# ontypehq/libfst

Hardware: AMD Instinct MI355X
Metric: strings/sec, compose_frozen_shortest_path_ambiguous len=64 batch=1M (higher is better)
Workload: dtype f64; 1 GPU; compose_frozen_shortest_path_ambiguous; semantics=eager, len=64, transducer_len=4096, branches=12, strings_per_gpu=1048576, global_batch=1048576, scaling_mode=weak: 1048576 strings per GPU per step, parallelism=dp1 (string shards, rhs replicated via RCCL broadcast)

## Files before the change

### libfst_amd/csrc/device_engine.hpp

```cpp
#pragma once

#include <hip/hip_runtime.h>

#include <atomic>
#include <condition_variable>
#include <cstdint>
#include <mutex>
#include <new>
#include <vector>

#include "fst_core.hpp"

namespace fstamd {

class FrozenFst;

constexpr uint32_t kSpanMixed = 0xFFFFFFFEu;
constexpr uint32_t kSpanNone = 0xFFFFFFFFu;
constexpr uint32_t kRecPad = 16;
constexpr uint32_t kDeadLabel = 0xFFFFFFFFu;

struct RhsView {
  const uint2* span;
  const double* final_w;
  const uint32_t* il;
  const ArcRec* rec;
  const uint4* sspan;
  uint32_t num_states;
  uint32_t num_arcs;
  uint32_t start;
  uint32_t max_span;
  uint32_t jump_back;
  uint32_t jump_fwd;
  const uint4* sspan2;
};

constexpr uint32_t kRevPos = 0x1000u;
struct RevRec {
  uint32_t src;
  uint32_t y;
  double weight;
};
static_assert(sizeof(RevRec) == 16, "RevRec is one 16-byte load");
struct RevView {
  const uint4* rspan;
  const uint4* gtab;
  const RevRec* rrec;
  const uint32_t* rolab;
  uint32_t kp;
  uint32_t gsearch;
  uint32_t direct;
  const uint4* rrec32;
  const uint2* rrec8;
  const uint32_t* rlab;
  const uint2* rxrec;
  uint32_t nrec;
  const uint32_t* rrec4;
  uint32_t rbias8;
  double winv;
};
constexpr uint32_t kPullWt = 64;
constexpr uint32_t kPullWtMax = 256;
__host__ __device__ inline const double* rv_weight_table(const RevView& rv) {
  return reinterpret_cast<const double*>(rv.rrec4 + ((rv.nrec + 1u) & ~1u));
}
constexpr double kRec8WMax = 7.0;

struct DeviceFst {
  int dev = 0;
  uint8_t* blob = nullptr;
  size_t blob_size = 0;
  uint2* span = nullptr;
  double* final_w = nullptr;
  uint32_t* il = nullptr;
  ArcRec* rec = nullptr;
  uint4* sspan = nullptr;
  RhsView view{};
  bool has_eps = false;
  bool nonneg = true;
  bool nan = false;
  bool finite = true;
  uint8_t weight_type = 0;
  bool pull_ok = false;
  bool lazy_pull_ok = false;
  double int_wmax = -1.0;
  bool widx = false;
  uint32_t wt_n = 0;
  bool byte_back = false;
  mutable std::atomic<int> skip_tiny_lazy{0}, skip_tiny_eager{0};
  mutable std::atomic<int> tiny_lazy_256{0}, tiny_eager_256{0};
  mutable std::atomic<uint64_t> tiny_lazy_seen{0}, tiny_lazy_over{0};
  RevView rev{};
  void* rev_bufs[9] = {};
  uint32_t* band_il = nullptr;
  ArcRec* band_rec = nullptr;
  uint32_t band_sh = 0;
  bool band_ol_sorted = false;
  std::vector<uint32_t> perm;

  static DeviceFst* create(const FrozenFst& f, int dev);
  static DeviceFst* adopt(const void* d_blob, const FrozenFst& host_view, int dev);
  static void destroy(DeviceFst* d);
};

struct BatchOutDev {
  int32_t* status;
  uint32_t* path_len;
  uint64_t* path_off;
  double* final_w;
  uint32_t* out_il;
  uint32_t* out_ol;
  double* out_w;
  uint64_t arc_cap;
  unsigned long long* cursor;
  uint32_t* work;
  const uint64_t* slots = nullptr;
  uint32_t* host_ol = nullptr;
  double* host_w = nullptr;
  int32_t* first_status = nullptr;
};

struct ChainInput {
  const uint32_t* labels;
  const uint64_t* offsets;
  uint32_t num_strings;
  uint32_t max_len;
};
struct GraphInput {
  const uint32_t* state_off;
  const uint32_t* arc_il;
  const uint32_t* arc_ol;
  const double* arc_w;
  const uint32_t* arc_next;
  const double* final_w;
  uint32_t num_states;
  uint32_t start;
  uint32_t max_outdeg;
  uint32_t ncap;
  uint32_t eps_out;
};

void* pin_host_alloc(size_t bytes);
void pin_host_release(void* p);
void device_pool_release(int dev);
template <class T>
struct PinnedAllocator {
  using value_type = T;
  PinnedAllocator() = default;
  template <class U>
  PinnedAllocator(const PinnedAllocator<U>&) {}
  T* allocate(size_t n) {
    void* p = pin_host_alloc(n * sizeof(T));
    if (!p) throw std::bad_alloc();
    return (T*)p;
  }
  void deallocate(T* p, size_t) { pin_host_release(p); }
  template <class U>
  bool operator==(const PinnedAllocator<U>&) const { return true; }
  template <class U>
  bool operator!=(const PinnedAllocator<U>&) const { return false; }
};
template <class T>
using PinnedVec = std::vector<T, PinnedAllocator<T>>;

struct HostLattice {
  int32_t status = 0;
  uint32_t n_nodes = 0, n_arcs = 0;
  PinnedVec<uint32_t> aoff, anext, ail, aol;
  PinnedVec<double> aw, nfin;
};
// ... 140 lines not shown
```

### libfst_amd/csrc/eager_pull.hip

```cpp
#include <algorithm>
#include <cmath>
#include <cstdio>
#include <cstdlib>
#include <cstring>
#include <unordered_map>
#include <vector>

#include "device_engine.hpp"
#include "host_fst.hpp"
#include "kernels/eager_pull.hpp"
#include "kernels/lazy_pull.hpp"

namespace fstamd {

namespace {

template <int KP, int WV, int RK>
const void* pull_kernel_ptr(bool direct) {
  return direct ? (const void*)eager_pull_kernel<kPullRows, KP, true, WV, RK>
                : (const void*)eager_pull_kernel<kPullRows, KP, false, WV, RK>;
}
#ifndef FSTAMD_PULL_WAVES_SMALL
#define FSTAMD_PULL_WAVES_SMALL 5
#endif
#ifndef FSTAMD_PULL_WAVES_F32
#define FSTAMD_PULL_WAVES_F32 6
#endif
#ifndef FSTAMD_PULL_WAVES_R8
#define FSTAMD_PULL_WAVES_R8 7
#endif
template <int RK>
const void* pull_kernel_for(const RevView& rv) {
  const bool dir = rv.direct != 0;
  constexpr int wv = RK == 5 ? 4
                   : RK == 4 ? FSTAMD_PULL_WAVES_SMALL
                   : RK >= 2 ? FSTAMD_PULL_WAVES_R8 : RK ? FSTAMD_PULL_WAVES_F32 : FSTAMD_PULL_WAVES_SMALL;
  switch (rv.kp) {
    case 4: return pull_kernel_ptr<4, wv, RK>(dir);
    case 5: return pull_kernel_ptr<5, wv, RK>(dir);
    default: return pull_kernel_ptr<8, 4, RK>(dir);
  }
}
bool use_rec8(const RevView& rv) { return rv.rrec8 && !std::getenv("FSTAMD_NO_REC8"); }
int route_rk(const char* sem, int rk, const RevView& rv, bool log) {
  if (log && std::getenv("FSTAMD_ROUTE_LOG"))
    std::fprintf(stderr, "[libfst_amd route] %s pull: records %d, weight scale %g\n", sem, rk,
                 rk && rk < 4 ? 1.0 / rv.winv : 1.0);
  return rk;
}
int pull_rk(const DeviceFst& rhs, uint32_t max_len) {
  if (!pull_f32(rhs, max_len) || std::getenv("FSTAMD_P_F64"))
    return rhs.rev.rrec4 && rhs.widx && !std::getenv("FSTAMD_NO_REC4")
               ? (rhs.wt_n <= kPullWt ? 4 : 5)
               : 0;
  if (rhs.rev.rrec4 && use_rec8(rhs.rev) && !std::getenv("FSTAMD_NO_REC4")) return 3;
  return use_rec8(rhs.rev) ? 2 : 1;
}
const void* pull_kernel_for(const DeviceFst& rhs, uint32_t max_len, bool log = false) {
  switch (route_rk("eager", pull_rk(rhs, max_len), rhs.rev, log)) {
    case 0: return pull_kernel_for<0>(rhs.rev);
    case 5: return pull_kernel_for<5>(rhs.rev);
    case 4: return pull_kernel_for<4>(rhs.rev);
    case 3: return pull_kernel_for<3>(rhs.rev);
    case 2: return pull_kernel_for<2>(rhs.rev);
    default: return pull_kernel_for<1>(rhs.rev);
  }
}
#ifndef FSTAMD_LP_WAVES_F32
#define FSTAMD_LP_WAVES_F32 5
#endif
#ifndef FSTAMD_LP_WAVES_F64
#define FSTAMD_LP_WAVES_F64 4
#endif
constexpr int kLazyPullWaves = 3;
template <int KP, int RK>
const void* lazy_pull_ptr(bool direct, bool b1) {
  constexpr int wv = KP > 5 ? kLazyPullWaves
                   : RK ? FSTAMD_LP_WAVES_F32 : FSTAMD_LP_WAVES_F64;
  if (!direct) return (const void*)lazy_pull_kernel<kPullRows, KP, false, wv, RK, false>;
  return b1 ? (const void*)lazy_pull_kernel<kPullRows, KP, true, wv, RK, true>
            : (const void*)lazy_pull_kernel<kPullRows, KP, true, wv, RK, false>;
}
template <int RK>
const void* lazy_pull_kernel_for(const DeviceFst& rhs) {
  const bool dir = rhs.rev.direct != 0, b1 = dir && rhs.byte_back;
  switch (rhs.rev.kp) {
    case 4: return lazy_pull_ptr<4, RK>(dir, b1);
    case 5: return lazy_pull_ptr<5, RK>(dir, b1);
    default: return lazy_pull_ptr<8, RK>(dir, b1);
  }
}
const void* lazy_pull_kernel_for(const DeviceFst& rhs, uint32_t max_len, bool log = false) {
  const int rk = !lazy_pull_f32(rhs, max_len) ? 0 : use_rec8(rhs.rev) ? 2 : 1;
  if (log && std::getenv("FSTAMD_ROUTE_LOG"))
    std::fprintf(stderr, "[libfst_amd route] lazy pull: back records %d B\n",
                 rhs.rev.direct && rhs.byte_back ? 1 : 4);
  switch (route_rk("lazy", rk, rhs.rev, log)) {
    case 0: return lazy_pull_kernel_for<0>(rhs);
    case 2: return lazy_pull_kernel_for<2>(rhs);
    default: return lazy_pull_kernel_for<1>(rhs);
  }
}
}

void free_reverse_mirror(DeviceFst* d) {
  for (void*& p : d->rev_bufs) {
    if (p) (void)hipFree(p);
    p = nullptr;
  }
  d->rev = RevView{};
  d->pull_ok = false;
  d->widx = false;
  d->wt_n = 0;
}

bool build_reverse_mirror(DeviceFst* d, const FrozenFst& f) {
  d->pull_ok = false;
  d->lazy_pull_ok = false;
  if (std::getenv("FSTAMD_NO_PULL")) return true;
  if (d->has_eps || !d->nonneg || d->nan) return true;
  const uint32_t ns = f.num_states(), na = f.header().num_arcs;
  if (ns == 0 || ns >= (1u << 27)) return true;
  const StateEntry* se = f.states();
  const PackedArc* pa = f.arcs();
  const std::vector<uint32_t>& perm = d->perm;
  auto pid = [&](uint32_t s) { return perm.empty() ? s : perm[s]; };

  std::vector<uint8_t> jpos(na);
  std::vector<uint32_t> src(na);
  std::vector<uint32_t> indeg(ns + 1, 0);
  for (uint32_t s = 0; s < ns; ++s) {
    uint32_t run = se[s].arc_offset;
    for (uint32_t a = se[s].arc_offset; a < se[s].arc_offset + se[s].num_arcs; ++a) {
      if (a > se[s].arc_offset && pa[a].ilabel != pa[a - 1].ilabel) run = a;
      if (a - run >= 8) return true;
      jpos[a] = (uint8_t)(a - run);
      src[a] = pid(s);
      ++indeg[pid(pa[a].nextstate)];
    }
  }
  bool ol_ordered = true;
  for (uint32_t s = 0; s < ns && ol_ordered; ++s)
    for (uint32_t a = se[s].arc_offset; a < se[s].arc_offset + se[s].num_arcs && ol_ordered; ++a)
      for (uint32_t b = a - jpos[a]; b < a; ++b)
        if (pa[b].nextstate == pa[a].nextstate && pa[b].olabel > pa[a].olabel) {
          ol_ordered = false;
          break;
        }
  std::vector<uint32_t> ioff(ns + 1, 0);
  for (uint32_t t = 0; t < ns; ++t) ioff[t + 1] = ioff[t] + indeg[t];
  std::vector<uint32_t> in(na), fill(ioff.begin(), ioff.end() - 1);
  for (uint32_t a = 0; a < na; ++a) in[fill[pid(pa[a].nextstate)]++] = a;
  for (uint32_t t = 0; t < ns; ++t)
    std::sort(in.begin() + ioff[t], in.begin() + ioff[t + 1], [&](uint32_t x, uint32_t y) {
      if (pa[x].ilabel != pa[y].ilabel) return pa[x].ilabel < pa[y].ilabel;
      if (src[x] != src[y]) return src[x] < src[y];
      return jpos[x] < jpos[y];
    });
  struct Group { uint32_t t, label, first, n; };
  std::vector<Group> groups;
  for (uint32_t t = 0; t < ns; ++t)
    for (uint32_t i = ioff[t]; i < ioff[t + 1];) {
      uint32_t e = i + 1;
      while (e < ioff[t + 1] && pa[in[e]].ilabel == pa[in[i]].ilabel) ++e;
      groups.push_back(Group{t, pa[in[i]].ilabel, i, e - i});
      i = e;
    }
  uint32_t kp = 8;
  uint64_t best_cost = ~0ull;
  for (uint32_t cand : {4u, 5u, 8u}) {
    uint64_t cost = 0;
    for (const Group& g : groups) {
      const uint64_t nb = (g.n + cand - 1) / cand;
      cost += nb * cand + (nb - 1) * cand;
    }
    if (cost < best_cost) {
      best_cost = cost;
      kp = cand;
    }
  }
  bool direct = !std::getenv("FSTAMD_PULL_INDIRECT");
  for (size_t g = 0; g < groups.size() && direct; ++g)
    if ((g > 0 && groups[g].t == groups[g - 1].t) || groups[g].label >= (1u << 24)) direct = false;
  const uint64_t ndirect = direct ? (uint64_t)ns + kPullW : 0;
  uint64_t nblocks = direct ? ndirect : 1;
  for (const Group& g : groups) nblocks += (g.n + kp - 1) / kp - (direct ? 1 : 0);
  if (nblocks * kp * sizeof(RevRec) > (4ull << 30) || nblocks * kp >= 0xFFFFFFFFull) return true;

  std::vector<RevRec> rrec(nblocks * kp, RevRec{0xFFFFFFF8u, 0u, 0.0});
  std::vector<uint32_t> rtgt(nblocks * kp, 0u);
  std::vector<uint32_t> rolab(nblocks * kp, 0u);
  std::vector<uint4> rspan((size_t)ns + kPullW, make_uint4(0u, 0u, kSpanNone, 0u));
  std::vector<uint4> gtab;
  uint32_t max_groups = 0;
  uint64_t blk = direct ? ndirect : 1;
  for (size_t gi = 0; gi < groups.size();) {
// ... 45 lines not shown
  for (uint32_t a = 0; a < na && d->int_wmax >= 0.0; ++a)
    d->int_wmax = std::max(d->int_wmax, pa[a].weight * wscale);
  if (wscale == 0.0) wscale = 1.0;
  auto wsc = [wscale](double w) { return (uint32_t)(w * wscale); };
  std::vector<uint32_t> rlab;
  std::vector<uint2> rxrec;
  if (direct) {
    rlab.resize(rspan.size());
    rxrec.resize(rspan.size());
    for (size_t t = 0; t < rspan.size(); ++t) {
      rlab[t] = (rspan[t].z & 0xFFFFFFu) | (std::min<uint32_t>(rspan[t].y, 255u) << 24);
      rxrec[t] = make_uint2(rspan[t].x, rspan[t].y);
    }
  }
  uint64_t max_nb = 0;
  for (const uint4& r : rspan)
    if (r.z != kSpanMixed) max_nb = std::max<uint64_t>(max_nb, r.y);
  const bool byte_back = direct && max_nb * kp <= 255 && !std::getenv("FSTAMD_NO_BYTE_BACK");
  std::vector<uint4> rrec32;
  std::vector<uint2> rrec8;
  if (d->int_wmax >= 0.0 && d->int_wmax <= kRec8WMax) {
    rrec8.resize(rrec.size());
    for (size_t r = 0; r < rrec.size(); ++r)
      rrec8[r] = make_uint2(rrec[r].src, rrec[r].y | wsc(rrec[r].weight));
  }
  std::vector<double> wtab;
  std::unordered_map<uint64_t, uint32_t> widx_of;
  if (d->int_wmax < 0.0 && !std::getenv("FSTAMD_NO_WIDX")) {
    bool ok = true;
    for (uint32_t a = 0; a < na && ok; ++a) {
      const double w = pa[a].weight;
      uint64_t bits;
      std::memcpy(&bits, &w, 8);
      if (widx_of.count(bits)) continue;
      if (!(w >= 0.0) || !std::isfinite(w) || wtab.size() == kPullWtMax) ok = false;
      else {
        widx_of.emplace(bits, (uint32_t)wtab.size());
        wtab.push_back(w);
      }
    }
    if (!ok) {
      wtab.clear();
      widx_of.clear();
    }
  }
  const bool widx = !wtab.empty();
  auto low_weight = [&](double w) -> uint32_t {
    if (!widx) return wsc(w);
    uint64_t bits;
    std::memcpy(&bits, &w, 8);
    return widx_of.at(bits);
  };
  std::vector<uint32_t> rrec4;
  uint32_t rbias8 = 0;
  if (!rrec8.empty() || widx) {
    int64_t dlo = 0, dhi = 0;
    for (size_t r = 0; r < rrec.size(); ++r) {
      if (rrec[r].src == 0xFFFFFFF8u) continue;
      const int64_t dl = (int64_t)rtgt[r] - (int64_t)(rrec[r].src >> 3);
      dlo = std::min(dlo, dl);
      dhi = std::max(dhi, dl);
    }
    if ((dhi - dlo) * 8 < 0xFFF0 && -dlo * 8 + 8 * (int64_t)kPullW <= 0xFFFF && byte_back) {
      rbias8 = (uint32_t)(-dlo * 8);
      rrec4.resize(rrec.size());
      for (size_t r = 0; r < rrec.size(); ++r) {
        const uint32_t y = rrec[r].y;
        if (rrec[r].src == 0xFFFFFFF8u) {
          rrec4[r] = 0xFFFF0000u;
        } else {
          const uint32_t low = (((y >> 17) & 7u) << 13) | (((y >> 13) & 15u) << 9) |
                               (((y >> 12) & 1u) << 8) | low_weight(rrec[r].weight);
          const int64_t dl = (int64_t)rtgt[r] - (int64_t)(rrec[r].src >> 3);
          rrec4[r] = ((uint32_t)((dl - dlo) * 8) << 16) | low;
        }
      }
    }
  }
  if (d->int_wmax >= 0.0) {
    rrec32.resize(rrec.size());
    for (size_t r = 0; r < rrec.size(); ++r)
      rrec32[r] = make_uint4(rrec[r].src, rrec[r].y, wsc(rrec[r].weight), rolab[r]);
  }
  if (rrec4.empty()) wtab.clear();
  if (!wtab.empty()) {
    d->wt_n = (uint32_t)wtab.size();
    wtab.resize(kPullWtMax, 0.0);
    rrec4.resize((rrec4.size() + 1) & ~(size_t)1, 0xFFFF0000u);
    const size_t at = rrec4.size();
    rrec4.resize(at + 2 * kPullWtMax);
    std::memcpy(rrec4.data() + at, wtab.data(), kPullWtMax * sizeof(double));
  }
  d->widx = !wtab.empty();
  auto up = [&](int i, const void* src_p, size_t bytes) -> bool {
    if (bytes == 0) bytes = 16;
    if (hipMalloc(&d->rev_bufs[i], bytes) != hipSuccess) return false;
    return hipMemcpy(d->rev_bufs[i], src_p, bytes, hipMemcpyHostToDevice) == hipSuccess;
  };
  const uint4 zero4 = make_uint4(0u, 0u, 0u, 0u);
  if (gtab.empty()) gtab.push_back(zero4);
  if (!up(0, rspan.data(), rspan.size() * sizeof(uint4)) ||
      !up(1, gtab.data(), gtab.size() * sizeof(uint4)) ||
      !up(2, rrec.data(), rrec.size() * sizeof(RevRec)) ||
      !up(3, rolab.data(), rolab.size() * sizeof(uint32_t)) ||
      (!rrec32.empty() && !up(4, rrec32.data(), rrec32.size() * sizeof(uint4))) ||
      (!rrec8.empty() && !up(5, rrec8.data(), rrec8.size() * sizeof(uint2))) ||
      (direct && (!up(6, rlab.data(), rlab.size() * sizeof(uint32_t)) ||
                  !up(7, rxrec.data(), rxrec.size() * sizeof(uint2)))) ||
      (!rrec4.empty() && !up(8, rrec4.data(), rrec4.size() * sizeof(uint32_t)))) {
    free_reverse_mirror(d);
    return false;
  }
  d->rev = RevView{(const uint4*)d->rev_bufs[0], (const uint4*)d->rev_bufs[1],
                   (const RevRec*)d->rev_bufs[2], (const uint32_t*)d->rev_bufs[3], kp, gsearch,
                   direct ? 1u : 0u, (const uint4*)d->rev_bufs[4], (const uint2*)d->rev_bufs[5],
                   (const uint32_t*)d->rev_bufs[6], (const uint2*)d->rev_bufs[7],
                   (uint32_t)(nblocks * kp), (const uint32_t*)d->rev_bufs[8], rbias8,
                   1.0 / wscale};
  d->byte_back = byte_back;
  d->pull_ok = true;
  d->lazy_pull_ok = ol_ordered && d->finite && !std::getenv("FSTAMD_NO_LAZY_PULL");
  return true;
}

bool pull_f32(const DeviceFst& rhs, uint32_t max_len) {
  return rhs.int_wmax >= 0.0 && rhs.rev.rrec32 && (double)max_len * rhs.int_wmax < 16777216.0;
}

int pull_waves_per_cu(const DeviceFst& rhs, uint32_t max_len) {
  int occ = 0;
  if (hipOccupancyMaxActiveBlocksPerMultiprocessor(&occ, pull_kernel_for(rhs, max_len), 64, 0) !=
      hipSuccess)
    occ = 1;
  return std::max(occ, 1);
}

hipError_t launch_eager_pull(const DeviceFst& rhs, const ChainInput& in, uint32_t n_best,
                             unsigned int* next_item, const EagerLaunch& lp,
                             const BatchOutDev& out, uint32_t grid, hipStream_t stream) {
  void* args[] = {(void*)&rhs.view, (void*)&rhs.rev, (void*)&in, (void*)&n_best,
                  (void*)&next_item, (void*)&lp, (void*)&out};
  return hipLaunchKernel(pull_kernel_for(rhs, in.max_len, true), dim3(grid), dim3(64), args, 0, stream);
}

bool lazy_pull_f32(const DeviceFst& rhs, uint32_t max_len) {
  return pull_f32(rhs, max_len) && rhs.int_wmax <= kLpF32WMax && !std::getenv("FSTAMD_LP_F64");
}

int lazy_pull_waves_per_cu(const DeviceFst& rhs, uint32_t max_len) {
  int occ = 0;
  if (hipOccupancyMaxActiveBlocksPerMultiprocessor(&occ, lazy_pull_kernel_for(rhs, max_len), 64, 0) !=
      hipSuccess)
    occ = 1;
  return std::max(occ, 1);
}

hipError_t launch_lazy_pull(const DeviceFst& rhs, const ChainInput& in, uint32_t n_best,
                            unsigned int* next_item, const EagerLaunch& lp,
                            const BatchOutDev& out, uint32_t grid, hipStream_t stream) {
  void* args[] = {(void*)&rhs.view, (void*)&rhs.rev, (void*)&in, (void*)&n_best,
                  (void*)&next_item, (void*)&lp, (void*)&out};
  return hipLaunchKernel(lazy_pull_kernel_for(rhs, in.max_len, true), dim3(grid), dim3(64), args, 0,
                         stream);
}

}
// ... 1 lines not shown
```

### libfst_amd/csrc/kernels/eager_pull.hpp

```cpp
#pragma once

#include <type_traits>

#include "device_common.hpp"
#include "eager_layered.hpp"
#include "eager_wave.hpp"
#include "eager_window.hpp"

namespace fstamd {

constexpr uint32_t kPullAbsent = 0xFFFF0000u;
#ifdef FSTAMD_P_TIGHT_SELECT
constexpr bool kTightSelect = true;
#else
constexpr bool kTightSelect = false;
#endif
constexpr uint32_t kDistAbsent = 0x7F000000u;
template <typename DT>
__device__ __forceinline__ DT dist_inf() {
  if constexpr (sizeof(DT) == 4) return (DT)kDistAbsent;
  else return (DT)__builtin_huge_val();
}
template <typename DT>
__device__ __forceinline__ DT dist_min(DT a, DT b) {
  if constexpr (sizeof(DT) == 4) return min(a, b);
  else return fmin(a, b);
}


template <int W, bool F32 = false, int WT = kPullWt>
struct PullLds {
  static constexpr int kWords = W * 8 / 64;
  double d[W + 1];
  unsigned long long rk[W + 1];
  unsigned long long bits[kWords];
  uint4 pre[kWords];
  unsigned long long best;
  uint32_t bestp;
  ChaseJob job[kChaseBatch];
  double wt[WT];
};
template <int W>
struct PullLds<W, true> {
  static constexpr int kWords = W * 8 / 64;
  uint2 cell[W + 1];
  unsigned long long bits[kWords];
  uint4 pre[kWords];
  unsigned long long best;
  uint32_t bestp;
  ChaseJob job[kChaseBatch];
};

template <int KP, typename DT>
__device__ __forceinline__ uint32_t tight_min(const DT (&nd)[KP], DT b, const uint32_t (&pk)[KP]) {
  uint32_t t[KP];
#pragma unroll
  for (int m = 0; m < KP; ++m) t[m] = nd[m] == b ? pk[m] : 0xFFFFFFFFu;
  uint32_t c = t[0];
#pragma unroll
  for (int m = 1; m < KP; m += 2) c = m + 1 < KP ? min(min(c, t[m]), t[m + 1]) : min(c, t[m]);
  return c;
}

template <typename T>
__device__ __forceinline__ const T* at_byte(const T* base, uint32_t byte_off) {
  return reinterpret_cast<const T*>(reinterpret_cast<const char*>(base) + byte_off);
}

template <int W>
__device__ __forceinline__ void pull_candidate(const PullLds<W>& S, const RevRec& r,
                                               uint32_t tmin8, uint32_t& pk, double& nd,
                                               uint32_t& rank_word) {
  const uint32_t off = min(r.src - tmin8, 8u * W);
  const double d = *reinterpret_cast<const double*>(reinterpret_cast<const char*>(S.d) + FB(off, 8 * (W + 1), 150));
  const uint32_t rw = *reinterpret_cast<const uint32_t*>(reinterpret_cast<const char*>(S.rk) + FB(off, 8 * (W + 1), 151));
  pk = rw | r.y | off;
  rank_word = rw;
  nd = d + r.weight;
}
template <int W, int WT>
__device__ __forceinline__ void pull_candidate(const PullLds<W, false, WT>& S, const uint32_t& r,
                                               uint32_t base8, uint32_t& pk, double& nd,
                                               uint32_t& rank_word) {
  const uint32_t off = min(base8 - (r >> 16), 8u * W);
  const double d = *reinterpret_cast<const double*>(reinterpret_cast<const char*>(S.d) + FB(off, 8 * (W + 1), 150));
  const uint32_t rw = *reinterpret_cast<const uint32_t*>(reinterpret_cast<const char*>(S.rk) + FB(off, 8 * (W + 1), 151));
  pk = rw | (r & 0xFFFFu);
  rank_word = rw;
  nd = d + S.wt[FB(r & (WT - 1u), WT, 149)];
}
template <int W>
__device__ __forceinline__ void pull_candidate(const PullLds<W, true>& S, const uint4& r,
                                               uint32_t tmin8, uint32_t& pk, uint32_t& nd,
                                               uint32_t& rank_word) {
  const uint32_t off = min(r.x - tmin8, 8u * W);
  const uint2 c = *reinterpret_cast<const uint2*>(reinterpret_cast<const char*>(S.cell) + FB(off, 8 * (W + 1), 152));
  pk = c.y | r.y | off;
  rank_word = c.y;
  nd = c.x + r.z;
}
__device__ __forceinline__ uint32_t rec8_weight(uint32_t y) { return y & 0xFFu; }
template <int W>
__device__ __forceinline__ void pull_candidate(const PullLds<W, true>& S, const uint2& r,
                                               uint32_t tmin8, uint32_t& pk, uint32_t& nd,
                                               uint32_t& rank_word) {
  const uint32_t off = min(r.x - tmin8, 8u * W);
  const uint2 c = *reinterpret_cast<const uint2*>(reinterpret_cast<const char*>(S.cell) + FB(off, 8 * (W + 1), 152));
  pk = c.y | r.y | off;
  rank_word = c.y;
  nd = c.x + rec8_weight(r.y);
}

template <int W>
__device__ __forceinline__ void pull_candidate(const PullLds<W, true>& S, const uint32_t& r,
                                               uint32_t base8, uint32_t& pk, uint32_t& nd,
                                               uint32_t& rank_word) {
  const uint32_t off = min(base8 - (r >> 16), 8u * W);
  const uint2 c = *reinterpret_cast<const uint2*>(reinterpret_cast<const char*>(S.cell) + FB(off, 8 * (W + 1), 152));
  pk = c.y | (r & 0xFFFFu);
  rank_word = c.y;
  nd = c.x + (r & 0xFFu);
}

__device__ __forceinline__ void pull_group(const RevView& rv, uint32_t lab, uint32_t t,
                                           uint32_t& rec0, uint32_t& nb) {
  const uint4 rs = rv.rspan[t];
  const bool hit = rs.z == lab && lab < kSpanMixed;
  rec0 = hit ? rs.x : 0u;
  nb = hit ? rs.y : 0u;
  if (rv.gsearch && __ballot(rs.z == kSpanMixed)) {
    if (rs.z == kSpanMixed) {
      uint32_t a = rs.x, b = rs.x + rs.y;
      for (uint32_t it = 0; it < rv.gsearch; ++it) {
        if (a < b) {
          const uint32_t mid = (a + b) >> 1;
          if (rv.gtab[mid].x < lab) a = mid + 1;
          else b = mid;
        }
      }
      if (a < rs.x + rs.y) {
        const uint4 g = rv.gtab[a];
        if (g.x == lab) {
          rec0 = g.y;
          nb = g.z;
        }
      }
    }
  }
}

template <int EW, int KP, bool DIRECT, int WAVES_PER_EU, int RK = 0>
__global__ void __launch_bounds__(64, WAVES_PER_EU)
eager_pull_kernel(RhsView rhs, RevView rv, ChainInput in, uint32_t n_best,
                  unsigned int* next_item, EagerLaunch lp, BatchOutDev out) {
  constexpr int W = 64 * EW;
  constexpr bool F32 = RK != 0 && RK != 4 && RK != 5;
  constexpr bool REC4 = RK >= 3;
  constexpr int WT = RK == 5 ? (int)kPullWtMax : (int)kPullWt;
  using DT = typename std::conditional<F32, uint32_t, double>::type;
  using RT = typename std::conditional<
      REC4, uint32_t,
      typename std::conditional<RK == 2, uint2,
                                typename std::conditional<F32, uint4, RevRec>::type>::type>::type;
  constexpr uint32_t kRankShift = REC4 ? 16 : 20;
  constexpr uint32_t kFirstShift = kRankShift - 3;
  constexpr uint32_t kMShift = kFirstShift - 4;
  constexpr int kWords = PullLds<W, F32, WT>::kWords;
  static_assert(KP <= 16, "m is 4 bits of the key");
  static_assert(W < 512, "8 * slot is 12 bits of the key, ranks 9 bits");
  __shared__ PullLds<W, F32, WT> S;
  const uint32_t lane = threadIdx.x;
  const DT kInf = dist_inf<DT>();
  auto set_cell = [&](uint32_t i, DT d, uint32_t rw) {
    if constexpr (F32) {
      S.cell[FB(i, W + 1, 153)] = make_uint2(d, rw);
    } else {
      S.d[FB(i, W + 1, 154)] = d;
      S.rk[FB(i, W + 1, 155)] = rw;
    }
  };
  auto rec = [&](uint32_t r) -> RT {
    if constexpr (REC4) return rv.rrec4[r];
    else if constexpr (RK == 2) return rv.rrec8[r];
    else if constexpr (F32) return rv.rrec32[r];
    else return rv.rrec[r];
  };
  uint2* const slabs = lp.back_ws + (size_t)blockIdx.x * kChaseBatch * lp.back_cap;
  uint32_t njobs = 0;

  auto chase_batch = [&]() {
    wave_lds_sync();
    uint32_t maxL = 0;
    ChaseJob jb{};
    if (lane < njobs) {
      jb = S.job[FB(lane, kChaseBatch, 156)];
      maxL = jb.L;
    }
    maxL = __builtin_amdgcn_readfirstlane(__ockl_wfred_max_u32(maxL));
    const uint32_t* sl = reinterpret_cast<const uint32_t*>(slabs + (size_t)lane * lp.back_cap);
    const uint2* hdr = slabs + (size_t)lane * lp.back_cap + lp.back_cap / 2;
    uint32_t id = jb.id;
    uint32_t tcur = jb.pad;
    for (uint32_t t = 0; t < maxL; ++t) {
      if (lane < njobs && t < jb.L) {
        const uint32_t k = jb.L - 1 - t;
        uint32_t b;
        if constexpr (REC4) {
          const uint32_t v = reinterpret_cast<const uint8_t*>(sl)[FB(id, lp.back_cap, 60)];
          b = FB(v < (uint32_t)KP ? tcur * KP + v : rv.rxrec[tcur].x + v - KP, rv.nrec, 63);
        } else {
          b = FB(sl[FB(id, lp.back_cap, 60)], rv.nrec, 63);
        }
        const uint2 h = hdr[k];
        if (!out.host_ol) out.out_il[jb.o + k] = in.labels[jb.off + k];
        uint32_t src8;
        if constexpr (REC4) {
          const uint32_t r = rv.rrec4[b];
          out.out_ol[jb.o + k] = rv.rolab[b];
          if constexpr (RK >= 4)
            out.out_w[jb.o + k] = rv_weight_table(rv)[r & (WT - 1u)];
          else
            out.out_w[jb.o + k] = (double)(r & 0xFFu) * rv.winv;
          tcur -= (uint32_t)(((int32_t)(r >> 16) - (int32_t)rv.rbias8) >> 3);
          src8 = tcur << 3;
        } else if constexpr (RK == 2) {
          const uint2 r = rv.rrec8[b];
          out.out_ol[jb.o + k] = rv.rolab[b];
          out.out_w[jb.o + k] = (double)rec8_weight(r.y) * rv.winv;
          src8 = r.x;
        } else if constexpr (F32) {
          const uint4 r = rv.rrec32[b];
          out.out_ol[jb.o + k] = r.w;
          out.out_w[jb.o + k] = (double)r.z * rv.winv;
          src8 = r.x;
        } else {
          const RevRec r = rv.rrec[b];
          out.out_ol[jb.o + k] = rv.rolab[b];
          out.out_w[jb.o + k] = r.weight;
          src8 = r.src;
        }
        id = h.x + ((src8 >> 3) - h.y);
      }
    }
    if (lane < njobs) {
      out.status[jb.si] = kPathOk;
      if (out.first_status) out.first_status[jb.si] = kPathOk;
      out.path_len[jb.si] = jb.L;
      out.path_off[jb.si] = jb.o;
      out.final_w[jb.si] = jb.fw;
      if (out.work) {
        out.work[2 * jb.si] = jb.tuples;
        out.work[2 * jb.si + 1] = jb.relax;
      }
    }
    if (out.host_ol) copy_out_paths(out, njobs, jb.o, jb.L, lane);
    njobs = 0;
    wave_lds_sync();
  };
  const uint32_t num_items = __builtin_amdgcn_readfirstlane(
      lp.num_items_dev ? *lp.num_items_dev : lp.num_items);
  const uint32_t want_work_w = __builtin_amdgcn_readfirstlane(out.work != nullptr ? 1u : 0u);
  auto want_work = [&]() -> bool {
    uint32_t w = __builtin_amdgcn_readfirstlane(want_work_w);
    asm volatile("" : "+s"(w));
    return w != 0u;
  };

#pragma unroll 1
  for (uint32_t i = lane; i < (uint32_t)W + 1; i += 64) set_cell(i, kInf, kPullAbsent);
  if (lane < (uint32_t)kWords) S.bits[FB(lane, kWords, 157)] = 0;
  if constexpr (RK >= 4)
    for (uint32_t i = lane; i < (uint32_t)WT; i += 64) S.wt[i] = rv_weight_table(rv)[i];
  wave_lds_sync();
  uint32_t wlast = 0;

  for (;;) {
    uint32_t item = 0;
    if (lane == 0) item = atomicAdd(next_item, 1u);
    item = __builtin_amdgcn_readfirstlane(item);
    if (item >= num_items) break;
    const uint32_t si = __builtin_amdgcn_readfirstlane(lp.items ? lp.items[item] : item);
    uint32_t* const back = reinterpret_cast<uint32_t*>(slabs + (size_t)njobs * lp.back_cap);
    uint2* const hdr = slabs + (size_t)njobs * lp.back_cap + lp.back_cap / 2;
    const uint64_t off0 = in.offsets[si];
    const uint64_t off = ((uint64_t)__builtin_amdgcn_readfirstlane((uint32_t)(off0 >> 32)) << 32) |
                         __builtin_amdgcn_readfirstlane((uint32_t)off0);
    const uint32_t L = __builtin_amdgcn_readfirstlane((uint32_t)(in.offsets[si + 1] - off));

    if (rhs.start == kNoState || n_best != 1) {
      if (lane == 0)
        write_status(out, si, (rhs.start == kNoState || n_best == 0) ? kPathEmpty : kPathErrorN,
                     0, 0);
      continue;
    }
    const unsigned long long t0 = __builtin_amdgcn_s_memrealtime();

#pragma unroll 1
    for (uint32_t i = lane; i < wlast; i += 64) set_cell(i, kInf, kPullAbsent);
    wave_lds_sync();
    if (lane == 0) set_cell(0, (DT)w_one(), 0u);
    wave_lds_sync();
    uint32_t tmin = rhs.start, wk = 1, base = 0, n_cur = 1;
    uint32_t cmin = rhs.start, cmax = rhs.start;
    uint32_t tuples = 1, relax = 0;
    int32_t fail = F32 && L > in.max_len ? kPathOverflow : kPathOk;
    unsigned long long mykey = kMaxU64;
    uint32_t myp = kEmptyKey;
    double myfw = 0.0;

    uint32_t labs = 0;
    for (uint32_t k = 0; k < L && fail == kPathOk; ++k) {
      if ((k & 15u) == 0 && __builtin_amdgcn_s_memrealtime() - t0 > lp.wd_ticks) {
        fail = kPathInternal;
        break;
      }
      if ((k & 63u) == 0) labs = k + lane < L ? in.labels[off + k + lane] : 0u;
      const uint32_t lab = __builtin_amdgcn_readlane(labs, k & 63u);
      if (lab == kEpsilon) {
        fail = kPathUnsupported;
        break;
      }
      const uint32_t tn = cmin >= rhs.jump_back ? cmin - rhs.jump_back : 0u;
      const uint32_t hi = min(cmax + rhs.jump_fwd, rhs.num_states - 1);
      const uint32_t nbase = base + wk;
      if (hi - tn >= (uint32_t)W || nbase + (hi - tn + 1) > lp.back_cap ||
          k >= lp.back_cap / 2) {
        fail = kPathOverflow;
        break;
      }
      const uint32_t wn = hi - tn + 1;
      const uint32_t rows_n = (wn + 63) / 64;

      uint32_t fst[EW], bk[EW], bra[EW];
      DT bd[EW];
#pragma unroll
      for (int e = 0; e < EW; ++e) {
        fst[e] = kEmptyKey;
        bk[e] = kEmptyKey;
        bra[e] = 0;
        bd[e] = kInf;
        if ((uint32_t)e >= rows_n) continue;
        const uint32_t i = (uint32_t)e * 64 + lane;
        const uint32_t t = tn + i;
        uint32_t rec0, nb, xrec = 0;
        uint32_t tmin8 = tmin << 3;
        if constexpr (DIRECT) {
          const uint32_t rs = *at_byte(rv.rlab, t * 4u);
          const bool hit = (rs & 0xFFFFFFu) == lab && lab < kSpanMixed;
          tmin8 = hit ? tmin8 : tmin8 + 0x80000000u;
          rec0 = t * KP;
          nb = hit ? rs >> 24 : 0u;
        } else {
          pull_group(rv, lab, t, rec0, nb);
        }
        if constexpr (REC4) tmin8 = (t << 3) - (tmin << 3) + rv.rbias8 + (tmin8 - (tmin << 3));
        RT rr[KP];
        const RT* R;
        if constexpr (REC4) R = at_byte(rv.rrec4, rec0 * 4u);
        else if constexpr (RK == 2) R = at_byte(rv.rrec8, rec0 * 8u);
        else if constexpr (F32) R = rv.rrec32 + rec0;
        else R = rv.rrec + rec0;
#pragma unroll
        for (int m = 0; m < KP; ++m) rr[m] = R[m];
        uint32_t pk[KP], rw[KP];
        DT nd[KP];
        uint32_t f = kEmptyKey;
        DT b = kInf;
        uint32_t c = kEmptyKey;
#pragma unroll
        for (int m = 0; m < KP; ++m) {
          pull_candidate<W>(S, rr[m], tmin8, pk[m], nd[m], rw[m]);
          f = min(f, pk[m]);
          b = dist_min(b, nd[m]);
        }
        if constexpr (F32 && !kTightSelect) {
#pragma unroll
          for (int m = 0; m < KP; ++m) c = min(c, pk[m] | ((b - nd[m]) & 0x80000000u));
        } else {
#pragma unroll
          for (int m = 0; m < KP; ++m) c = min(c, nd[m] == b ? pk[m] : kEmptyKey);
        }
        if (want_work()) {
#pragma unroll
          for (int m = 0; m < KP; ++m) relax += (uint32_t)__popcll(__ballot(rw[m] < kPullAbsent));
        }
        uint32_t ra = (REC4 ? 0u : rec0) + ((c >> kMShift) & 15u);
        if (__ballot(nb > 1)) {
          if constexpr (DIRECT) {
            const uint2 xr = nb > 1 ? rv.rxrec[t] : make_uint2(0u, nb);
            xrec = xr.x;
            nb = xr.y;
          }
          for (uint32_t x = 1;; ++x) {
            const bool act = nb > x;
            if (!__ballot(act)) break;
            const uint32_t rx = act ? (DIRECT ? xrec + (x - 1) * KP : rec0 + x * KP)
                                    : (DIRECT ? rhs.num_states * KP : 0u);
#pragma unroll
            for (int m = 0; m < KP; ++m) {
              uint32_t p2, w2;
              DT n2;
              pull_candidate<W>(S, rec(rx + m), tmin8, p2, n2, w2);
              f = min(f, p2);
              if (n2 < b || (n2 == b && p2 < c)) {
                b = n2;
                c = p2;
                ra = REC4 ? x * KP + m : rx + m;
              }
              if (want_work()) relax += (uint32_t)__popcll(__ballot(w2 < kPullAbsent));
            }
          }
        }
        fst[e] = f;
        bd[e] = b;
        bk[e] = c;
        bra[e] = ra;
        if (f < kPullAbsent) {
          const uint32_t key = f >> kFirstShift;
          atomicOr(reinterpret_cast<uint32_t*>(S.bits) + FB(key >> 5, 2 * kWords, 158), 1u << (key & 31u));
        }
      }
      wave_lds_sync();

      const uint32_t nw = (n_cur * 8 + 63) / 64;
      unsigned long long word = 0;
      if (lane < nw) word = S.bits[FB(lane, kWords, 159)];
      const uint32_t pc = (uint32_t)__popcll(word);
      const uint32_t inc = wave_incl_scan_dpp(pc);
      const uint32_t n_next = __builtin_amdgcn_readlane(inc, 63);
      if (lane < nw) {
        S.pre[FB(lane, kWords, 160)] = make_uint4(inc - pc, (uint32_t)word,
                                 inc - pc + (uint32_t)__popc((uint32_t)word), (uint32_t)(word >> 32));
        S.bits[FB(lane, kWords, 161)] = 0;
      }
      wave_lds_sync();
      if (n_next == 0) {
        n_cur = 0;
        break;
      }

      const bool last = k + 1 == L;
      if (lane == 0) hdr[k] = make_uint2(base, tmin);
      const uint32_t rows_w = max(rows_n, (wk + 63) / 64);
      uint32_t lo_slot = kEmptyKey, hi_slot = 0;
#pragma unroll
      for (int e = 0; e < EW; ++e) {
        if ((uint32_t)e >= rows_w) continue;
        const uint32_t i = (uint32_t)e * 64 + lane;
        if ((uint32_t)e >= rows_n) {
          set_cell(i, bd[e], kPullAbsent);
          continue;
        }
        uint32_t fe = fst[e];
        asm volatile("" : "+v"(fe));
        const bool pres = fe < kPullAbsent;
        const uint32_t key = pres ? fe >> kFirstShift : 0u;
        const uint2 p = reinterpret_cast<const uint2*>(S.pre)[FB(key >> 5, 2 * kWords, 162)];
        const uint32_t rank = p.x + (uint32_t)__popc(p.y & ((1u << (key & 31u)) - 1u));
        set_cell(i, bd[e], pres ? rank << kRankShift : kPullAbsent);
        const unsigned long long pm = __ballot(pres);
        if (pm) {
          lo_slot = min(lo_slot, (uint32_t)e * 64 + (uint32_t)__builtin_ctzll(pm));
          hi_slot = max(hi_slot, (uint32_t)e * 64 + 63u - (uint32_t)__builtin_clzll(pm));
        }
        if (pres) {
          if constexpr (REC4)
            reinterpret_cast<uint8_t*>(back)[FB(nbase + i, lp.back_cap, 61)] = (uint8_t)bra[e];
          else
            *const_cast<uint32_t*>(at_byte(back, FB(nbase + i, lp.back_cap, 61) * 4u)) = bra[e];
          if (last) {
            const uint32_t t = tn + i;
            const double fw2 = rhs.final_w[FB(t, rhs.num_states, 62)];
            if (!w_is_zero((double)bd[e]) && !w_is_zero(fw2)) {
              const unsigned long long kk = okey((double)bd[e] * (F32 ? rv.winv : 1.0) + fw2);
              const uint32_t pp = (rank << 9) | i;
              if (kk < mykey || (kk == mykey && pp < myp)) {
                mykey = kk;
                myp = pp;
                myfw = fw2;
              }
            }
          }
        }
      }
      tmin = tn;
      base = nbase;
      wk = wn;
      n_cur = n_next;
      tuples += n_next;
      cmin = tn + lo_slot;
      cmax = tn + hi_slot;
      wave_lds_sync();
    }
    wlast = wk;

    if (fail != kPathOk) {
      if (lane == 0) write_status(out, si, fail, tuples, relax);
      continue;
    }
    if (L == 0 && lane == 0) {
      const double fw2 = rhs.final_w[rhs.start];
      if (!w_is_zero(fw2)) {
        mykey = okey(w_one() + fw2);
        myp = 0;
        myfw = fw2;
      }
    }
    uint32_t bp;
    double fw2;
    if (n_cur == 0 || !wave_pick_best(S.best, S.bestp, lane, mykey, myp, myfw, bp, fw2)) {
      if (lane == 0) write_status(out, si, kPathEmpty, tuples, relax);
      continue;
    }
    unsigned long long o = 0;
    if (lane == 0) o = reserve_path(out, si, L);
    o = ((unsigned long long)__builtin_amdgcn_readfirstlane((uint32_t)(o >> 32)) << 32) |
        __builtin_amdgcn_readfirstlane((uint32_t)o);
    if (o + L > out.arc_cap) {
      if (lane == 0) write_status(out, si, kPathOutputFull, tuples, relax);
      continue;
    }
    if (lane == 0) {
      ChaseJob& j = S.job[FB(njobs, kChaseBatch, 163)];
      j.si = si;
      j.L = L;
      j.id = base + (bp & 511u);
      j.pad = tmin + (bp & 511u);
      j.tuples = tuples;
      j.relax = relax;
      j.o = o;
      j.off = off;
      j.fw = fw2;
    }
    if (++njobs == (uint32_t)kChaseBatch) chase_batch();
  }
  if (njobs) chase_batch();
}

}
```

Baseline: 35.17 million strings/s.

## Add packed 32-bit cell/record path for eager pull relaxation

Adds an RK=6 packed variant of the eager pull kernel. It stores distance and rank together in one 32-bit LDS cell and builds a repacked record array in which a single 24-bit mad yields a combined distance/rank/m key, so one integer min does the selection. The goal is fewer LDS accesses and fewer ALU ops per candidate relaxation, with records loaded before the label check. It applies only when weights are integer-scaled, the layout is direct, kp < 15, and the path cost fits in 15 bits. It also adds a second copy of the records in device memory.

```diff
diff --git a/libfst_amd/csrc/device_engine.hpp b/libfst_amd/csrc/device_engine.hpp
--- a/libfst_amd/csrc/device_engine.hpp
+++ b/libfst_amd/csrc/device_engine.hpp
@@ -63,6 +63,9 @@
 constexpr uint32_t kPullWtMax = 256;
 __host__ __device__ inline const double* rv_weight_table(const RevView& rv) {
   return reinterpret_cast<const double*>(rv.rrec4 + ((rv.nrec + 1u) & ~1u));
+}
+__host__ __device__ inline const uint32_t* rv_packed(const RevView& rv) {
+  return rv.rrec4 + ((rv.nrec + 1u) & ~1u);
 }
 constexpr double kRec8WMax = 7.0;
 
@@ -86,6 +89,7 @@
   double int_wmax = -1.0;
   bool widx = false;
   uint32_t wt_n = 0;
+  bool pack = false;
   bool byte_back = false;
   mutable std::atomic<int> skip_tiny_lazy{0}, skip_tiny_eager{0};
   mutable std::atomic<int> tiny_lazy_256{0}, tiny_eager_256{0};
diff --git a/libfst_amd/csrc/eager_pull.hip b/libfst_amd/csrc/eager_pull.hip
--- a/libfst_amd/csrc/eager_pull.hip
+++ b/libfst_amd/csrc/eager_pull.hip
@@ -29,16 +29,27 @@
 #ifndef FSTAMD_PULL_WAVES_R8
 #define FSTAMD_PULL_WAVES_R8 7
 #endif
+#ifndef FSTAMD_PULL_WAVES_PACK
+#define FSTAMD_PULL_WAVES_PACK FSTAMD_PULL_WAVES_R8
+#endif
 template <int RK>
 const void* pull_kernel_for(const RevView& rv) {
   const bool dir = rv.direct != 0;
-  constexpr int wv = RK == 5 ? 4
-                   : RK == 4 ? FSTAMD_PULL_WAVES_SMALL
-                   : RK >= 2 ? FSTAMD_PULL_WAVES_R8 : RK ? FSTAMD_PULL_WAVES_F32 : FSTAMD_PULL_WAVES_SMALL;
-  switch (rv.kp) {
-    case 4: return pull_kernel_ptr<4, wv, RK>(dir);
-    case 5: return pull_kernel_ptr<5, wv, RK>(dir);
-    default: return pull_kernel_ptr<8, 4, RK>(dir);
+  if constexpr (RK == 6) {
+    switch (rv.kp) {
+      case 4: return (const void*)eager_pull_kernel<kPullRows, 4, true, FSTAMD_PULL_WAVES_PACK, 6>;
+      case 5: return (const void*)eager_pull_kernel<kPullRows, 5, true, FSTAMD_PULL_WAVES_PACK, 6>;
+      default: return (const void*)eager_pull_kernel<kPullRows, 8, true, 4, 6>;
+    }
+  } else {
+    constexpr int wv = RK == 5 ? 4
+                     : RK == 4 ? FSTAMD_PULL_WAVES_SMALL
+                     : RK >= 2 ? FSTAMD_PULL_WAVES_R8 : RK ? FSTAMD_PULL_WAVES_F32 : FSTAMD_PULL_WAVES_SMALL;
+    switch (rv.kp) {
+      case 4: return pull_kernel_ptr<4, wv, RK>(dir);
+      case 5: return pull_kernel_ptr<5, wv, RK>(dir);
+      default: return pull_kernel_ptr<8, 4, RK>(dir);
+    }
   }
 }
 bool use_rec8(const RevView& rv) { return rv.rrec8 && !std::getenv("FSTAMD_NO_REC8"); }
@@ -56,8 +67,19 @@
   if (rhs.rev.rrec4 && use_rec8(rhs.rev) && !std::getenv("FSTAMD_NO_REC4")) return 3;
   return use_rec8(rhs.rev) ? 2 : 1;
 }
+bool pull_pack(const DeviceFst& rhs, uint32_t max_len) {
+  return rhs.pack && pull_rk(rhs, max_len) == 3 &&
+         ((double)max_len + 1.0) * rhs.int_wmax < (double)0x7F00 && !std::getenv("FSTAMD_NO_PACK");
+}
 const void* pull_kernel_for(const DeviceFst& rhs, uint32_t max_len, bool log = false) {
-  switch (route_rk("eager", pull_rk(rhs, max_len), rhs.rev, log)) {
+  const int rk = route_rk("eager", pull_rk(rhs, max_len), rhs.rev, log);
+  if (rk == 3) {
+    const bool pack = pull_pack(rhs, max_len);
+    if (log && std::getenv("FSTAMD_ROUTE_LOG"))
+      std::fprintf(stderr, "[libfst_amd route] eager pull: packed cells %s\n", pack ? "on" : "off");
+    if (pack) return pull_kernel_for<6>(rhs.rev);
+  }
+  switch (rk) {
     case 0: return pull_kernel_for<0>(rhs.rev);
     case 5: return pull_kernel_for<5>(rhs.rev);
     case 4: return pull_kernel_for<4>(rhs.rev);
@@ -112,6 +134,7 @@
   d->pull_ok = false;
   d->widx = false;
   d->wt_n = 0;
+  d->pack = false;
 }
 
 bool build_reverse_mirror(DeviceFst* d, const FrozenFst& f) {
@@ -323,6 +346,25 @@
     for (size_t r = 0; r < rrec.size(); ++r)
       rrec32[r] = make_uint4(rrec[r].src, rrec[r].y, wsc(rrec[r].weight), rolab[r]);
   }
+  bool pack = !rrec4.empty() && !widx && !rrec8.empty() && kp < 15 && rbias8 % 8 == 0;
+  for (size_t g = 0; g < groups.size() && pack; ++g) pack = groups[g].label != 0xFFFFFFu;
+  for (size_t r = 0; r < rrec4.size() && pack; ++r)
+    pack = rrec4[r] == 0xFFFF0000u || (rrec4[r] >> 16) / 2 <= 252;
+  if (pack) {
+    const size_t n = rrec4.size();
+    rrec4.resize(((n + 1) & ~(size_t)1) + n, 0xFFFF0000u);
+    uint32_t* const rpk = rrec4.data() + ((n + 1) & ~(size_t)1);
+    for (size_t r = 0; r < n; ++r) {
+      const uint32_t v = rrec4[r];
+      if (v == 0xFFFF0000u) {
+        const size_t first = r - r % kp;
+        rpk[r] = first < r && rrec4[first] != 0xFFFF0000u ? (rpk[first] & ~15u) | 15u : 15u;
+      } else {
+        rpk[r] = ((v >> 17) << 24) | ((v & 0xFFu) << 16) | (((v >> 13) & 7u) << 4) | ((v >> 9) & 15u);
+      }
+    }
+  }
+  d->pack = pack;
   if (rrec4.empty()) wtab.clear();
   if (!wtab.empty()) {
     d->wt_n = (uint32_t)wtab.size();
diff --git a/libfst_amd/csrc/kernels/eager_pull.hpp b/libfst_amd/csrc/kernels/eager_pull.hpp
--- a/libfst_amd/csrc/kernels/eager_pull.hpp
+++ b/libfst_amd/csrc/kernels/eager_pull.hpp
@@ -51,6 +51,28 @@
   ChaseJob job[kChaseBatch];
 };
 
+constexpr uint32_t kPackAbsent = 0x7F00FF80u;
+constexpr uint32_t kPackNoRank = 0xFF80u;
+constexpr uint32_t kPackPadM = 15u;
+template <int W>
+struct PullLdsPacked {
+  static constexpr int kWords = W * 8 / 64;
+  uint32_t cell[W + 1];
+  unsigned long long bits[kWords];
+  uint4 pre[kWords];
+  unsigned long long best;
+  uint32_t bestp;
+  ChaseJob job[kChaseBatch];
+};
+__device__ __forceinline__ uint32_t pack_candidate(uint32_t r, uint32_t c) {
+  uint32_t cand;
+  asm("v_mad_u32_u24 %0, %1, 1, %2" : "=v"(cand) : "v"(r), "v"(c));
+  return cand;
+}
+__device__ __forceinline__ bool pack_counts(uint32_t cand) {
+  return (cand & 0xFFFFu) < kPackNoRank && (cand & 15u) != kPackPadM;
+}
+
 template <int KP, typename DT>
 __device__ __forceinline__ uint32_t tight_min(const DT (&nd)[KP], DT b, const uint32_t (&pk)[KP]) {
   uint32_t t[KP];
@@ -156,23 +178,30 @@
   constexpr int W = 64 * EW;
   constexpr bool F32 = RK != 0 && RK != 4 && RK != 5;
   constexpr bool REC4 = RK >= 3;
+  constexpr bool PACK = RK == 6;
+  static_assert(!PACK || (DIRECT && KP < (int)kPackPadM), "packed cells: direct layout, m = 15 is padding");
   constexpr int WT = RK == 5 ? (int)kPullWtMax : (int)kPullWt;
   using DT = typename std::conditional<F32, uint32_t, double>::type;
   using RT = typename std::conditional<
       REC4, uint32_t,
       typename std::conditional<RK == 2, uint2,
                                 typename std::conditional<F32, uint4, RevRec>::type>::type>::type;
-  constexpr uint32_t kRankShift = REC4 ? 16 : 20;
+  constexpr uint32_t kRankShift = PACK ? 7 : REC4 ? 16 : 20;
   constexpr uint32_t kFirstShift = kRankShift - 3;
   constexpr uint32_t kMShift = kFirstShift - 4;
-  constexpr int kWords = PullLds<W, F32, WT>::kWords;
+  using LdsT = typename std::conditional<PACK, PullLdsPacked<W>, PullLds<W, F32, WT>>::type;
+  constexpr int kWords = LdsT::kWords;
+  constexpr uint32_t kAbsent = PACK ? kPackNoRank : kPullAbsent;
   static_assert(KP <= 16, "m is 4 bits of the key");
   static_assert(W < 512, "8 * slot is 12 bits of the key, ranks 9 bits");
-  __shared__ PullLds<W, F32, WT> S;
+  __shared__ LdsT S;
   const uint32_t lane = threadIdx.x;
-  const DT kInf = dist_inf<DT>();
+  const DT kInf = PACK ? (DT)(kPackAbsent >> 16) : dist_inf<DT>();
+  const uint32_t* const rpk = PACK ? rv_packed(rv) : nullptr;
   auto set_cell = [&](uint32_t i, DT d, uint32_t rw) {
-    if constexpr (F32) {
+    if constexpr (PACK) {
+      S.cell[FB(i, W + 1, 153)] = ((uint32_t)d << 16) | rw;
+    } else if constexpr (F32) {
       S.cell[FB(i, W + 1, 153)] = make_uint2(d, rw);
     } else {
       S.d[FB(i, W + 1, 154)] = d;
@@ -180,7 +209,8 @@
     }
   };
   auto rec = [&](uint32_t r) -> RT {
-    if constexpr (REC4) return rv.rrec4[r];
+    if constexpr (PACK) return rpk[r];
+    else if constexpr (REC4) return rv.rrec4[r];
     else if constexpr (RK == 2) return rv.rrec8[r];
     else if constexpr (F32) return rv.rrec32[r];
     else return rv.rrec[r];
@@ -214,7 +244,13 @@
         const uint2 h = hdr[k];
         if (!out.host_ol) out.out_il[jb.o + k] = in.labels[jb.off + k];
         uint32_t src8;
-        if constexpr (REC4) {
+        if constexpr (PACK) {
+          const uint32_t r = rpk[b];
+          out.out_ol[jb.o + k] = rv.rolab[b];
+          out.out_w[jb.o + k] = (double)((r >> 16) & 0xFFu) * rv.winv;
+          tcur = tcur - (r >> 26) + (rv.rbias8 >> 3);
+          src8 = tcur << 3;
+        } else if constexpr (REC4) {
           const uint32_t r = rv.rrec4[b];
           out.out_ol[jb.o + k] = rv.rolab[b];
           if constexpr (RK >= 4)
@@ -267,9 +303,9 @@
   };
 
 #pragma unroll 1
-  for (uint32_t i = lane; i < (uint32_t)W + 1; i += 64) set_cell(i, kInf, kPullAbsent);
+  for (uint32_t i = lane; i < (uint32_t)W + 1; i += 64) set_cell(i, kInf, kAbsent);
   if (lane < (uint32_t)kWords) S.bits[FB(lane, kWords, 157)] = 0;
-  if constexpr (RK >= 4)
+  if constexpr (RK == 4 || RK == 5)
     for (uint32_t i = lane; i < (uint32_t)WT; i += 64) S.wt[i] = rv_weight_table(rv)[i];
   wave_lds_sync();
   uint32_t wlast = 0;
@@ -296,7 +332,7 @@
     const unsigned long long t0 = __builtin_amdgcn_s_memrealtime();
 
 #pragma unroll 1
-    for (uint32_t i = lane; i < wlast; i += 64) set_cell(i, kInf, kPullAbsent);
+    for (uint32_t i = lane; i < wlast; i += 64) set_cell(i, kInf, kAbsent);
     wave_lds_sync();
     if (lane == 0) set_cell(0, (DT)w_one(), 0u);
     wave_lds_sync();
@@ -344,45 +380,76 @@
         const uint32_t t = tn + i;
         uint32_t rec0, nb, xrec = 0;
         uint32_t tmin8 = tmin << 3;
+        RT rr[KP];
         if constexpr (DIRECT) {
           const uint32_t rs = *at_byte(rv.rlab, t * 4u);
-          const bool hit = (rs & 0xFFFFFFu) == lab && lab < kSpanMixed;
+          if constexpr (PACK) {
+            const uint32_t* const R = at_byte(rpk, t * (4u * KP));
+#pragma unroll
+            for (int m = 0; m < KP; ++m) rr[m] = R[m];
+            __builtin_amdgcn_sched_barrier(0);
+          }
+          const bool hit = (rs & 0xFFFFFFu) == lab && lab < (PACK ? 0xFFFFFFu : kSpanMixed);
           tmin8 = hit ? tmin8 : tmin8 + 0x80000000u;
           rec0 = t * KP;
           nb = hit ? rs >> 24 : 0u;
         } else {
           pull_group(rv, lab, t, rec0, nb);
         }
-        if constexpr (REC4) tmin8 = (t << 3) - (tmin << 3) + rv.rbias8 + (tmin8 - (tmin << 3));
-        RT rr[KP];
-        const RT* R;
-        if constexpr (REC4) R = at_byte(rv.rrec4, rec0 * 4u);
-        else if constexpr (RK == 2) R = at_byte(rv.rrec8, rec0 * 8u);
-        else if constexpr (F32) R = rv.rrec32 + rec0;
-        else R = rv.rrec + rec0;
-#pragma unroll
-        for (int m = 0; m < KP; ++m) rr[m] = R[m];
+        if constexpr (PACK) tmin8 = (t << 2) - (tmin << 2) + (rv.rbias8 >> 1) + (tmin8 - (tmin << 3));
+        else if constexpr (REC4) tmin8 = (t << 3) - (tmin << 3) + rv.rbias8 + (tmin8 - (tmin << 3));
+        if constexpr (!PACK) {
+          const RT* R;
+          if constexpr (REC4) R = at_byte(rv.rrec4, rec0 * 4u);
+          else if constexpr (RK == 2) R = at_byte(rv.rrec8, rec0 * 8u);
+          else if constexpr (F32) R = rv.rrec32 + rec0;
+          else R = rv.rrec + rec0;
+#pragma unroll
+          for (int m = 0; m < KP; ++m) rr[m] = R[m];
+        }
         uint32_t pk[KP], rw[KP];
         DT nd[KP];
         uint32_t f = kEmptyKey;
         DT b = kInf;
         uint32_t c = kEmptyKey;
-#pragma unroll
-        for (int m = 0; m < KP; ++m) {
-          pull_candidate<W>(S, rr[m], tmin8, pk[m], nd[m], rw[m]);
-          f = min(f, pk[m]);
-          b = dist_min(b, nd[m]);
-        }
-        if constexpr (F32 && !kTightSelect) {
-#pragma unroll
-          for (int m = 0; m < KP; ++m) c = min(c, pk[m] | ((b - nd[m]) & 0x80000000u));
+        if constexpr (PACK) {
+#pragma unroll
+          for (int m = 0; m < KP; ++m) {
+            const uint32_t off = min(tmin8 - (rr[m] >> 24), 4u * W);
+            rw[m] = *reinterpret_cast<const uint32_t*>(reinterpret_cast<const char*>(S.cell) + FB(off, 4 * (W + 1), 152));
+          }
+#pragma unroll
+          for (int m = 0; m < KP; ++m) pk[m] = pack_candidate(rr[m], rw[m]);
+          uint16_t f16 = (uint16_t)pk[0];
+          c = pk[0];
+#pragma unroll
+          for (int m = 1; m < KP; ++m) {
+            c = min(c, pk[m]);
+            f16 = __builtin_elementwise_min(f16, (uint16_t)pk[m]);
+          }
+          f = f16;
+          if (want_work()) {
+#pragma unroll
+            for (int m = 0; m < KP; ++m) relax += (uint32_t)__popcll(__ballot(pack_counts(pk[m])));
+          }
         } else {
 #pragma unroll
-          for (int m = 0; m < KP; ++m) c = min(c, nd[m] == b ? pk[m] : kEmptyKey);
-        }
-        if (want_work()) {
-#pragma unroll
-          for (int m = 0; m < KP; ++m) relax += (uint32_t)__popcll(__ballot(rw[m] < kPullAbsent));
+          for (int m = 0; m < KP; ++m) {
+            pull_candidate<W>(S, rr[m], tmin8, pk[m], nd[m], rw[m]);
+            f = min(f, pk[m]);
+            b = dist_min(b, nd[m]);
+          }
+          if constexpr (F32 && !kTightSelect) {
+#pragma unroll
+            for (int m = 0; m < KP; ++m) c = min(c, pk[m] | ((b - nd[m]) & 0x80000000u));
+          } else {
+#pragma unroll
+            for (int m = 0; m < KP; ++m) c = min(c, nd[m] == b ? pk[m] : kEmptyKey);
+          }
+          if (want_work()) {
+#pragma unroll
+            for (int m = 0; m < KP; ++m) relax += (uint32_t)__popcll(__ballot(rw[m] < kPullAbsent));
+          }
         }
         uint32_t ra = (REC4 ? 0u : rec0) + ((c >> kMShift) & 15u);
         if (__ballot(nb > 1)) {
@@ -398,16 +465,31 @@
                                     : (DIRECT ? rhs.num_states * KP : 0u);
 #pragma unroll
             for (int m = 0; m < KP; ++m) {
-              uint32_t p2, w2;
-              DT n2;
-              pull_candidate<W>(S, rec(rx + m), tmin8, p2, n2, w2);
-              f = min(f, p2);
-              if (n2 < b || (n2 == b && p2 < c)) {
-                b = n2;
-                c = p2;
-                ra = REC4 ? x * KP + m : rx + m;
+              if constexpr (PACK) {
+                const uint32_t r2 = rec(rx + m);
+                const uint32_t off = min(tmin8 - (r2 >> 24), 4u * W);
+                const uint32_t cl = *reinterpret_cast<const uint32_t*>(reinterpret_cast<const char*>(S.cell) + FB(off, 4 * (W + 1), 152));
+                const uint32_t p2 = pack_candidate(r2, cl);
+                if (act) {
+                  f = min(f, p2 & 0xFFFFu);
+                  if (p2 < c) {
+                    c = p2;
+                    ra = x * KP + m;
+                  }
+                }
+                if (want_work()) relax += (uint32_t)__popcll(__ballot(act && pack_counts(p2)));
+              } else {
+                uint32_t p2, w2;
+                DT n2;
+                pull_candidate<W>(S, rec(rx + m), tmin8, p2, n2, w2);
+                f = min(f, p2);
+                if (n2 < b || (n2 == b && p2 < c)) {
+                  b = n2;
+                  c = p2;
+                  ra = REC4 ? x * KP + m : rx + m;
+                }
+                if (want_work()) relax += (uint32_t)__popcll(__ballot(w2 < kPullAbsent));
               }
-              if (want_work()) relax += (uint32_t)__popcll(__ballot(w2 < kPullAbsent));
             }
           }
         }
@@ -415,7 +497,7 @@
         bd[e] = b;
         bk[e] = c;
         bra[e] = ra;
-        if (f < kPullAbsent) {
+        if (f < kAbsent) {
           const uint32_t key = f >> kFirstShift;
           atomicOr(reinterpret_cast<uint32_t*>(S.bits) + FB(key >> 5, 2 * kWords, 158), 1u << (key & 31u));
         }
@@ -448,16 +530,19 @@
         if ((uint32_t)e >= rows_w) continue;
         const uint32_t i = (uint32_t)e * 64 + lane;
         if ((uint32_t)e >= rows_n) {
-          set_cell(i, bd[e], kPullAbsent);
+          set_cell(i, bd[e], kAbsent);
           continue;
         }
         uint32_t fe = fst[e];
         asm volatile("" : "+v"(fe));
-        const bool pres = fe < kPullAbsent;
+        const bool pres = fe < kAbsent;
         const uint32_t key = pres ? fe >> kFirstShift : 0u;
         const uint2 p = reinterpret_cast<const uint2*>(S.pre)[FB(key >> 5, 2 * kWords, 162)];
         const uint32_t rank = p.x + (uint32_t)__popc(p.y & ((1u << (key & 31u)) - 1u));
-        set_cell(i, bd[e], pres ? rank << kRankShift : kPullAbsent);
+        if constexpr (PACK)
+          S.cell[FB(i, W + 1, 153)] = (bk[e] & 0xFFFF0000u) | (pres ? rank << kRankShift : kAbsent);
+        else
+          set_cell(i, bd[e], pres ? rank << kRankShift : kPullAbsent);
         const unsigned long long pm = __ballot(pres);
         if (pm) {
           lo_slot = min(lo_slot, (uint32_t)e * 64 + (uint32_t)__builtin_ctzll(pm));
@@ -471,8 +556,9 @@
           if (last) {
             const uint32_t t = tn + i;
             const double fw2 = rhs.final_w[FB(t, rhs.num_states, 62)];
-            if (!w_is_zero((double)bd[e]) && !w_is_zero(fw2)) {
-              const unsigned long long kk = okey((double)bd[e] * (F32 ? rv.winv : 1.0) + fw2);
+            const DT de = PACK ? (DT)(bk[e] >> 16) : bd[e];
+            if (!w_is_zero((double)de) && !w_is_zero(fw2)) {
+              const unsigned long long kk = okey((double)de * (F32 ? rv.winv : 1.0) + fw2);
               const uint32_t pp = (rank << 9) | i;
               if (kk < mykey || (kk == mykey && pp < myp)) {
                 mykey = kk;
```

Result: faster. 37.22 million strings/s, median of 6 (+5.8%).
